# warlock-labs/sylow

Hardware: AMD Instinct MI355X
Metric: BN254 pairings/s (value) and BLS verifies/s (config.bls_verifies_per_s) at batch=2^20 per GPU (higher is better)
Workload: dtype i32/u32 limbs (9x29-bit carry-free core + 8x32-bit Montgomery, exact integer)

## Files before the change

sylow_amd/csrc/bn254_pair29.hpp:

```cpp
#pragma once
#include "bn254_f29.hpp"
#include "bn254_pair.hpp"

namespace bn254 {
namespace pl {

struct W2 { F29 c; };
BN_DEV const F29& f29_of(const W2& a) { return a.c; }
BN_DEV F29& f29_of(W2& a) { return a.c; }
struct W6 { W2 c0, c1, c2; };
struct W12 { W6 c0, c1; };

BN_DEV F29 xchg9(const F29& a) {
  F29 r;
#pragma unroll
  for (int i = 0; i < 9; ++i) r.v[i] = (i32)swap_u32((u32)a.v[i]);
  return r;
}
BN_DEV F29 sel9(bool odd, const F29& if_even, const F29& if_odd) {
  F29 r;
#pragma unroll
  for (int i = 0; i < 9; ++i) r.v[i] = odd ? if_odd.v[i] : if_even.v[i];
  return r;
}
// ... 124 lines not shown
BN_DEV W2 w2_xi_lin(const W2& x, int k, const W2& y, int m) {
  const F29 xo = xchg9(x.c);
  if (m == 0) {
    const F29* const t[2] = {&x.c, &xo};
    const i32 c[2] = {bn_keep(9 * k), bn_keep_v(lane_odd() ? k : -k)};
    return W2{f29_reduce_terms(t, c)};
  }
  const F29* const t[3] = {&x.c, &xo, &y.c};
  const i32 c[3] = {bn_keep(9 * k), bn_keep_v(lane_odd() ? k : -k), bn_keep(m)};
  return W2{f29_reduce_terms(t, c)};
}

BN_DEV W2 w2_from_s2(const S2& a) { return W2{f29_reduce(f29_from_fp(a.c))}; }
BN_DEV S2 w2_to_s2(const W2& a) { return S2{f29_to_fp(a.c)}; }
BN_DEV W2 w2_const(const uint32_t (&c)[2][8]) { return w2_from_s2(s2_const(c)); }
BN_DEV void w12_from_s12(W12& r, const S12& a) {
  r.c0.c0 = w2_from_s2(a.c0.c0); r.c0.c1 = w2_from_s2(a.c0.c1); r.c0.c2 = w2_from_s2(a.c0.c2);
  r.c1.c0 = w2_from_s2(a.c1.c0); r.c1.c1 = w2_from_s2(a.c1.c1); r.c1.c2 = w2_from_s2(a.c1.c2);
}
BN_DEV void w12_to_s12(S12& r, const W12& a) {
  r.c0.c0 = w2_to_s2(a.c0.c0); r.c0.c1 = w2_to_s2(a.c0.c1); r.c0.c2 = w2_to_s2(a.c0.c2);
  r.c1.c0 = w2_to_s2(a.c1.c0); r.c1.c1 = w2_to_s2(a.c1.c1); r.c1.c2 = w2_to_s2(a.c1.c2);
}

struct W6Raw { W2 v0, x0, y1, v2, y2; };
template <bool INL = false> BN_DEV W2 w2_mul_sel(const W2& a, const W2& b) { return INL ? w2_mul_inl(a, b) : w2_mul(a, b); }
template <bool INL = false>
BN_DEV W6Raw w6_mul_raw(const W6& a, const W6& b) {
  W2 v0, v1, v2, s0, s1, s2;
  W2_MUL2_SEL(INL, v0, v1, a.c0, b.c0, a.c1, b.c1);
  W2_MUL2_SEL(INL, v2, s0, a.c2, b.c2, w2_sub(a.c1, a.c2), w2_sub(b.c1, b.c2));
  W2_MUL2_SEL(INL, s1, s2, w2_sub(a.c0, a.c1), w2_sub(b.c0, b.c1), w2_sub(a.c0, a.c2), w2_sub(b.c0, b.c2));
  return W6Raw{v0, w2_sub(w2_add(v1, v2), s0), w2_sub(w2_add(v0, v1), s1), v2, w2_add(w2_sub(w2_add(v0, v2), s2), v1)};
}
template <bool INL = false>
BN_DEV W6 w6_mul(const W6& a, const W6& b) {
  const W6Raw m = w6_mul_raw<INL>(a, b);
  W6 r;
  r.c0 = w2_xi_lin(m.x0, 1, m.v0, 1);
  r.c1 = w2_xi_lin(m.v2, 1, m.y1, 1);
  r.c2 = w2_reduce(m.y2);
  return r;
}
BN_DEV W6 w6_add_norm(const W6& a, const W6& b) {
  return W6{w2_norm(w2_add(a.c0, b.c0)), w2_norm(w2_add(a.c1, b.c1)), w2_norm(w2_add(a.c2, b.c2))};
}
BN_DEV W6 w6_sub(const W6& a, const W6& b) { return W6{w2_sub(a.c0, b.c0), w2_sub(a.c1, b.c1), w2_sub(a.c2, b.c2)}; }

BN_DEV void w12_mul_c1(W12& r, const W6Raw& t2, const W6& t0, const W6& t1) {
  r.c1.c0 = w2_xi_lin(t2.x0, 1, w2_sub(w2_sub(t2.v0, t0.c0), t1.c0), 1);
  r.c1.c1 = w2_xi_lin(t2.v2, 1, w2_sub(w2_sub(t2.y1, t0.c1), t1.c1), 1);
  r.c1.c2 = w2_lin2(w2_sub(t2.y2, t0.c2), 1, t1.c2, -1);
}
BN_DEV W12 w12_mul(const W12& a, const W12& b) {
  const W6 t0 = w6_mul(a.c0, b.c0);
  const W6 t1 = w6_mul(a.c1, b.c1);
  const W6Raw t2 = w6_mul_raw(w6_add_norm(a.c0, a.c1), w6_add_norm(b.c0, b.c1));
  W12 r;
  w12_mul_c1(r, t2, t0, t1);
  r.c0.c0 = w2_xi_lin(t1.c2, 1, t0.c0, 1);
  r.c0.c1 = w2_norm(w2_add(t0.c1, t1.c0));
  r.c0.c2 = w2_norm(w2_add(t0.c2, t1.c1));
  return r;
}
BN_DEV W6 w6_mul_b2zero(const W6& a, const W6& b) {
  W2 v0, v1, p21, p20;
  W2_MUL2(v0, v1, a.c0, b.c0, a.c1, b.c1);
  W2_MUL2(p21, p20, a.c2, b.c1, a.c2, b.c0);
  const W2 s1 = w2_mul(w2_sub(a.c0, a.c1), w2_sub(b.c0, b.c1));
  W6 r;
  r.c0 = w2_xi_lin(p21, 1, v0, 1);
  r.c1 = w2_reduce(w2_sub(w2_add(v0, v1), s1));
  r.c2 = w2_norm(w2_add(p20, v1));
  return r;
}
BN_DEV W12 w12_mul_line_pair(const W12& a, const W12& b) {
  const W6 t0 = w6_mul(a.c0, b.c0);
  const W6 t1 = w6_mul_b2zero(a.c1, b.c1);
  const W6Raw t2 = w6_mul_raw(w6_add_norm(a.c0, a.c1), W6{w2_norm(w2_add(b.c0.c0, b.c1.c0)), w2_norm(w2_add(b.c0.c1, b.c1.c1)), b.c0.c2});
  W12 r;
  w12_mul_c1(r, t2, t0, t1);
  r.c0.c0 = w2_xi_lin(t1.c2, 1, t0.c0, 1);
  r.c0.c1 = w2_norm(w2_add(t0.c1, t1.c0));
  r.c0.c2 = w2_norm(w2_add(t0.c2, t1.c1));
  return r;
}
template <bool INL = false>
BN_DEV W12 w12_sqr(const W12& a) {
  const W6 d{w2_norm(w2_sub(a.c0.c0, a.c1.c0)), w2_norm(w2_sub(a.c0.c1, a.c1.c1)), w2_norm(w2_sub(a.c0.c2, a.c1.c2))};
  W6 e;
  e.c0 = w2_xi_lin(a.c1.c2, -1, a.c0.c0, 1);
  e.c1 = w2_norm(w2_sub(a.c0.c1, a.c1.c0));
  e.c2 = w2_norm(w2_sub(a.c0.c2, a.c1.c1));
  const W6 c2 = w6_mul<INL>(a.c0, a.c1);
  const W6Raw m = w6_mul_raw<INL>(d, e);
  W12 r;
  r.c1.c0 = w2_norm(w2_add(c2.c0, c2.c0));
  r.c1.c1 = w2_norm(w2_add(c2.c1, c2.c1));
  r.c1.c2 = w2_norm(w2_add(c2.c2, c2.c2));
  r.c0.c0 = w2_xi_lin(w2_add(m.x0, c2.c2), 1, w2_add(m.v0, c2.c0), 1);
  {
    const F29 xo = xchg9(m.v2.c);
    const W2 cc = w2_add(c2.c1, c2.c0);
    const F29* const t[4] = {&m.v2.c, &xo, &m.y1.c, &cc.c};
    const i32 c[4] = {bn_keep(9), bn_keep_v(lane_odd() ? 1 : -1), bn_keep(1), bn_keep(1)};
    r.c0.c1 = W2{f29_reduce_terms(t, c)};
  }
  r.c0.c2 = w2_lin2(m.y2, 1, w2_add(c2.c2, c2.c1), 1);
  return r;
}
BN_DEV W12 w12_conj(const W12& a) {
  W12 r;
  r.c0 = a.c0;
  r.c1.c0 = w2_norm(w2_neg(a.c1.c0)); r.c1.c1 = w2_norm(w2_neg(a.c1.c1)); r.c1.c2 = w2_norm(w2_neg(a.c1.c2));
  return r;
}
BN_DEV W2 w2_conj(const W2& a) { return W2{sel9(lane_odd(), a.c, f29_norm(f29_neg(a.c)))}; }
template <int E>
BN_DEV W6 w6_frobenius(const W6& a) {
  constexpr bool oddE = (E & 1) != 0;
  const uint32_t (&k1)[2][8] = (E == 1) ? C_FROB6_C1_1 : (E == 2) ? C_FROB6_C1_2 : C_FROB6_C1_3;
  const uint32_t (&k2)[2][8] = (E == 1) ? C_FROB6_C2_1 : (E == 2) ? C_FROB6_C2_2 : C_FROB6_C2_3;
  W6 r;
  r.c0 = oddE ? w2_conj(a.c0) : a.c0;
  W2_MUL2(r.c1, r.c2, oddE ? w2_conj(a.c1) : a.c1, w2_const(k1), oddE ? w2_conj(a.c2) : a.c2, w2_const(k2));
  return r;
}
template <int E>
BN_DEV W12 w12_frobenius(const W12& a) {
  const uint32_t (&k)[2][8] = (E == 1) ? C_FROB12_C1_1 : (E == 2) ? C_FROB12_C1_2 : C_FROB12_C1_3;
  const W2 kk = w2_const(k);
  const W6 x1 = w6_frobenius<E>(a.c1);
  W6 y;
  W2_MUL2(y.c0, y.c1, x1.c0, kk, x1.c1, kk);
  y.c2 = w2_mul(x1.c2, kk);
  return W12{w6_frobenius<E>(a.c0), y};
}
BN_DEV W12 w12_sparse_mul(const W12& f, const W2& x0, const W2& x4, const W2& x2) {
  const W2 z0 = f.c0.c0, z1 = f.c0.c1, z2 = f.c0.c2, z3 = f.c1.c0, z4 = f.c1.c1, z5 = f.c1.c2;
  W2 d0, d2, d4, p12, p54, p10, p34, p30, p52, q02, q24, q04;
  W2_MUL2(d0, d2, z0, x0, z2, x2);
  W2_MUL2(d4, p12, z4, x4, z1, x2);
  W2_MUL2(p54, p10, z5, x4, z1, x0);
  W2_MUL2(p34, p30, z3, x4, z3, x0);
  W2_MUL2(p52, q02, z5, x2, w2_sub(z0, z2), w2_sub(x0, x2));
  W2_MUL2(q24, q04, w2_sub(z2, z4), w2_sub(x2, x4), w2_sub(z0, z4), w2_sub(x0, x4));
  const W2 qs = w2_mul(w2_norm(w2_add(w2_add(z1, z3), z5)), w2_norm(w2_add(w2_add(x0, x2), x4)));
  W12 o;
  o.c0.c0 = w2_xi_lin(w2_add(p12, d4), 1, d0, 1);
  o.c0.c1 = w2_xi_lin(w2_add(p54, d2), 1, p10, 1);
  o.c0.c2 = w2_reduce(w2_add(w2_sub(w2_add(d0, d2), q02), p34));
  o.c1.c0 = w2_xi_lin(w2_sub(w2_add(d2, d4), q24), 1, p30, 1);
  o.c1.c1 = w2_xi_lin(p52, 1, w2_sub(w2_add(d0, d4), q04), 1);
  {
    const W2 sa = w2_add(w2_add(p12, p54), p10), sb = w2_add(w2_add(p34, p30), p52);
    const F29* const t[3] = {&qs.c, &sa.c, &sb.c};
    const i32 c[3] = {bn_keep(1), bn_keep(-1), bn_keep(-1)};
    o.c1.c2 = W2{f29_reduce_terms(t, c)};
  }
  return o;
}
BN_DEV W2 w2_xi_lin_v(const W2& x, const W2& y, i32 m) {
  const F29 xo = xchg9(x.c);
  const F29* const t[3] = {&x.c, &xo, &y.c};
  const i32 c[3] = {bn_keep(9), bn_keep_v(lane_odd() ? 1 : -1), bn_keep_v(m)};
  return W2{f29_reduce_terms(t, c)};
}
BN_DEV W2 w2_lin_v(const W2& x, const W2& y, i32 m) {
  const F29* const t[2] = {&x.c, &y.c};
  const i32 c[2] = {bn_keep(1), bn_keep_v(m)};
  return W2{f29_reduce_terms(t, c)};
}
BN_DEV W12 w12_sparse_mul_unit(const W12& f, i32 u, const W2& x4, const W2& x2) {
  const W2 z0 = f.c0.c0, z1 = f.c0.c1, z2 = f.c0.c2, z3 = f.c1.c0, z4 = f.c1.c1, z5 = f.c1.c2;
  W2 d2, d4, p12, p54, p34, p52, a02, a04, q24, q13;
  W2_MUL2(d2, d4, z2, x2, z4, x4);
  W2_MUL2(p12, p54, z1, x2, z5, x4);
  W2_MUL2(p34, p52, z3, x4, z5, x2);
  W2_MUL2(a02, a04, z0, x2, z0, x4);
  const W2 x24 = w2_sub(x2, x4);
  W2_MUL2(q24, q13, w2_sub(z2, z4), x24, w2_sub(z1, z3), x24);
  W12 o;
  o.c0.c0 = w2_xi_lin_v(w2_add(p12, d4), z0, u);
  o.c0.c1 = w2_xi_lin_v(w2_add(p54, d2), z1, u);
  o.c0.c2 = w2_lin_v(w2_add(a02, p34), z2, u);
  o.c1.c0 = w2_xi_lin_v(w2_sub(w2_add(d2, d4), q24), z3, u);
  {
    const F29 xo = xchg9(p52.c);
    const F29* const t[4] = {&p52.c, &xo, &a04.c, &z4.c};
    const i32 c[4] = {bn_keep(9), bn_keep_v(lane_odd() ? 1 : -1), bn_keep(1), bn_keep_v(u)};
    o.c1.c1 = W2{f29_reduce_terms(t, c)};
  }
  o.c1.c2 = w2_lin_v(w2_sub(w2_add(p12, p34), q13), z5, u);
  return o;
}
BN_DEV W2 w2_xi_norm(const W2& x, const W2& y) {
  const F29 xo = xchg9(x.c);
  const F29* const t[3] = {&x.c, &xo, &y.c};
  const i32 c[3] = {bn_keep(9), bn_keep_v(lane_odd() ? 1 : -1), bn_keep(1)};
  return W2{f29_norm_terms(t, c)};
}
BN_DEV W2 w2_xi_norm_sub(const W2& x, const W2& y) {
  const F29 xo = xchg9(x.c);
  const F29* const t[3] = {&x.c, &xo, &y.c};
  const i32 c[3] = {bn_keep(-9), bn_keep_v(lane_odd() ? -1 : 1), bn_keep(1)};
  return W2{f29_norm_terms(t, c)};
}
template <bool INL = false>
BN_DEV void w_fp4_square_fold(W2& out0, W2& m, const W2& a, const W2& b, const W2& z) {
  W2 w;
  W2_MUL2_SEL(INL, m, w, a, b, w2_sub(a, b), w2_xi_norm_sub(b, a));
  const F29 mo = xchg9(m.c);
  const F29* const t[4] = {&w.c, &m.c, &mo, &z.c};
  const i32 c[4] = {bn_keep(3), bn_keep(30), bn_keep_v(lane_odd() ? 3 : -3), bn_keep(-2)};
  out0 = W2{f29_reduce_terms(t, c)};
}
template <bool INL = false>
BN_DEV W12 w12_cyclotomic_sqr(const W12& f) {
  const W2 z0 = f.c0.c0, z4 = f.c0.c1, z3 = f.c0.c2, z2 = f.c1.c0, z1 = f.c1.c1, z5 = f.c1.c2;
  W2 m;
  W12 r;
  w_fp4_square_fold<INL>(r.c0.c0, m, z0, z1, z0);
  r.c1.c1 = w2_lin2(m, 6, z1, 2);
  w_fp4_square_fold<INL>(r.c0.c1, m, z2, z3, z4);
  r.c1.c2 = w2_lin2(m, 6, z5, 2);
  w_fp4_square_fold<INL>(r.c0.c2, m, z4, z5, z3);
  r.c1.c0 = w2_xi_lin(m, 6, z2, 2);
  return r;
}

BN_DEV F29 f29_halve(const F29& a) {
  i32 p[9]; f29_p(p);
  const i32 m = -(a.v[0] & 1);
  i32 lo[9];
  i32 c = 0;
#pragma unroll
  for (int i = 0; i < 8; ++i) {
    i32 t = a.v[i] + (p[i] & m) + c;
    lo[i] = t & BN_M29;
    c = t >> 29;
  }
  lo[8] = a.v[8] + (p[8] & m) + c;
  F29 r;
#pragma unroll
  for (int i = 0; i < 8; ++i) r.v[i] = (lo[i] >> 1) | ((lo[i + 1] & 1) << 28);
  r.v[8] = lo[8] >> 1;
  return r;
}
BN_DEV W2 w2_halve(const W2& a) { return W2{f29_halve(a.c)}; }
BN_DEV W2 w2_triple(const W2& a) { return W2{f29_add(f29_add(a.c, a.c), a.c)}; }
struct G2W { W2 x, y, z; };
BN_DEV W2 w2_twist_b() {
  const F29 k0{{0x12cb9911, 0x1fcb719e, 0x1368f727, 0x1ff96726, 0x0aadc75b, 0x179b4484, 0x06475c9b, 0x020e578d, -1520355}};
  const F29 k1{{0x0322ef99, 0x06e86c1b, 0x13f74e78, 0x0a0a4222, 0x0bcef269, 0x0af6e9ff, 0x0644c3a7, 0x0acd7c01, -535829}};
  return W2{sel9(lane_odd(), k0, k1)};
}
BN_DEV F29 f29_iso_s2() { return F29{{0x05beeef0, 0x1f76bf90, 0x1d5e46cf, 0x17f6764e, 0x1df385e5, 0x0d7a8334, 0x152215eb, 0x01b6eac1, -290196}}; }
BN_DEV F29 f29_iso_s3() { return F29{{0x1af1f8a3, 0x00cd9858, 0x1dce6a34, 0x142e620a, 0x1bc0c667, 0x0ae94d20, 0x0db9310b, 0x12572b72, 0x000405e6}}; }
BN_DEV W2 w2_mul_27m3u(const W2& a) {
  const F29 ao = xchg9(a.c);
  const F29* const t[2] = {&a.c, &ao};
  const i32 c[2] = {bn_keep(27), bn_keep_v(lane_odd() ? -3 : 3)};
  return W2{f29_reduce_terms(t, c)};
}
template <bool ISO = false>
BN_DEV void g2_doubling_step29(G2W& r, W2& l0, W2& l1, W2& l2) {
#if BN_QUAD
  W2 xy, xx, b, c, yz2, e;
  W2_MUL_SQR(xy, xx, r.x, r.y, r.x);
  const W2 a = w2_halve(xy);
  l2 = w2_norm(w2_triple(xx));
  W2_SQR2(b, c, r.y, r.z);
  if (ISO) {
    yz2 = w2_sqr(w2_norm(w2_add(r.y, r.z)));
    e = w2_mul_27m3u(c);
  } else {
    W2_SQR_MUL(yz2, e, w2_norm(w2_add(r.y, r.z)), w2_twist_b(), w2_norm(w2_triple(c)));
  }
  const W2 h = w2_norm(w2_sub(yz2, w2_add(b, c)));
  l1 = w2_neg(h);
  l0 = w2_xi_lin(w2_sub(e, b), 1, b, 0);
  const W2 f = w2_norm(w2_triple(e));
  W2_MUL2(r.z, r.x, b, h, a, w2_sub(b, f));
  const W2 g = w2_halve(w2_norm(w2_add(b, f)));
  W2 gg, ee;
  W2_SQR2(gg, ee, g, e);
  r.y = w2_lin2(gg, 1, ee, -3);
#else
  const W2 a = w2_halve(w2_mul(r.x, r.y));
  l2 = w2_norm(w2_triple(w2_sqr(r.x)));
  const W2 b = w2_sqr(r.y);
  const W2 c = w2_sqr(r.z);
  const W2 h = w2_norm(w2_sub(w2_sqr(w2_norm(w2_add(r.y, r.z))), w2_add(b, c)));
  const W2 e = ISO ? w2_mul_27m3u(c) : w2_mul(w2_twist_b(), w2_norm(w2_triple(c)));
  l1 = w2_neg(h);
  r.z = w2_mul(b, h);
  l0 = w2_xi_lin(w2_sub(e, b), 1, b, 0);
  const W2 f = w2_norm(w2_triple(e));
  r.x = w2_mul(a, w2_sub(b, f));
  const W2 g = w2_halve(w2_norm(w2_add(b, f)));
  r.y = w2_lin2(w2_sqr(g), 1, w2_sqr(e), -3);
#endif
}
BN_DEV void g2_addition_step29(G2W& r, const W2& bx, const W2& by, W2& l0, W2& l1, W2& l2) {
#if BN_QUAD
  W2 zbx, zby, ebx, dby;
  W2_MUL2(zbx, zby, r.z, bx, r.z, by);
  const W2 d = w2_sub(r.x, zbx);
  const W2 e = w2_sub(r.y, zby);
  W2_MUL2(ebx, dby, e, bx, d, by);
  l0 = w2_xi_lin(w2_sub(ebx, dby), 1, bx, 0);
  l1 = d;
  l2 = w2_neg(e);
  const W2 dn = w2_norm(d), en = w2_norm(e);
  W2 f, ee, h, i, zee, zh, dj, hy;
  W2_SQR2(f, ee, dn, en);
  W2_MUL2(h, i, dn, f, r.x, f);
  W2_MUL2(zee, zh, r.z, ee, r.z, h);
  const W2 j = w2_norm(w2_sub(w2_add(zee, h), w2_add(i, i)));
  W2_MUL2(dj, hy, dn, j, h, r.y);
  r.z = zh;
  r.x = dj;
  r.y = w2_norm(w2_sub(w2_mul(en, w2_sub(i, j)), hy));
#else
  const W2 d = w2_sub(r.x, w2_mul(r.z, bx));
  const W2 e = w2_sub(r.y, w2_mul(r.z, by));
  l0 = w2_xi_lin(w2_sub(w2_mul(e, bx), w2_mul(d, by)), 1, bx, 0);
  l1 = d;
  l2 = w2_neg(e);
  const W2 dn = w2_norm(d), en = w2_norm(e);
  const W2 f = w2_sqr(dn);
  const W2 h = w2_mul(dn, f);
  const W2 i = w2_mul(r.x, f);
  const W2 j = w2_norm(w2_sub(w2_add(w2_mul(r.z, w2_sqr(en)), h), w2_add(i, i)));
  r.z = w2_mul(r.z, h);
  r.x = w2_mul(dn, j);
  r.y = w2_norm(w2_sub(w2_mul(en, w2_sub(i, j)), w2_mul(h, r.y)));
#endif
}
BN_DEV W12 w12_line_product(const W2& a0, const W2& a4, const W2& a2, const W2& b0, const W2& b4, const W2& b2) {
  W2 d0, d2, d4, k02, k24, k04;
  W2_MUL2(d0, d2, a0, b0, a2, b2);
  W2_MUL2(d4, k02, a4, b4, w2_sub(a0, a2), w2_sub(b0, b2));
  W2_MUL2(k24, k04, w2_sub(a2, a4), w2_sub(b2, b4), w2_sub(a0, a4), w2_sub(b0, b4));
  W12 r;
  r.c0.c0 = w2_xi_lin(d4, 1, d0, 1);
  r.c0.c1 = w2_xi_lin(d2, 1, d2, 0);
  r.c0.c2 = w2_reduce(w2_sub(w2_add(d0, d2), k02));
  r.c1.c0 = w2_xi_lin(w2_sub(w2_add(d2, d4), k24), 1, d2, 0);
  r.c1.c1 = w2_reduce(w2_sub(w2_add(d0, d4), k04));
  r.c1.c2 = W2{F29{{0, 0, 0, 0, 0, 0, 0, 0, 0}}};
  return r;
}
constexpr int MILLER_LDS_WORDS = 36, MILLER_LDS_WORDS_PARK = 63;
BN_DEV void lds_put9(i32 (*lds)[256], int slot, const F29& a) {
#pragma unroll
  for (int i = 0; i < 9; ++i) lds[9 * slot + i][threadIdx.x] = a.v[i];
}
BN_DEV F29 lds_get9(i32 (*lds)[256], int slot) {
  F29 r;
#pragma unroll
  for (int i = 0; i < 9; ++i) r.v[i] = lds[9 * slot + i][threadIdx.x];
  return r;
}
#ifndef BN_MILLER_SQR_INL
#define BN_MILLER_SQR_INL false
#endif
template <bool PARK, bool ISO = false>
BN_NOINLINE void miller_loop29g(S12& fout, const Fp& pxs, const Fp& pys, const S2& qxs_in, const S2& qys_in) {
  __shared__ i32 lds[PARK ? MILLER_LDS_WORDS_PARK : MILLER_LDS_WORDS][256];
  S2 qxs = qxs_in, qys = qys_in;
  {
    const F29 px = f29_reduce(f29_from_fp(pxs)), py = f29_reduce(f29_from_fp(pys));
    lds_put9(lds, 0, ISO ? f29_mul(px, f29_iso_s2()) : px);
    lds_put9(lds, 1, ISO ? f29_mul(py, f29_iso_s3()) : py);
  }
  {
    W2 qx = w2_from_s2(qxs), qy = w2_from_s2(qys);
    if (ISO) {
      W2_SCALE2(qx, qy, qx, f29_iso_s2(), qy, f29_iso_s3());
      qxs = w2_to_s2(qx); qys = w2_to_s2(qy);
    }
    lds_put9(lds, 2, qx.c);
    lds_put9(lds, 3, qy.c);
  }
  auto PX = [&]() { return lds_get9(lds, 0); };
  auto PY = [&]() { return lds_get9(lds, 1); };
  auto QX = [&]() { return W2{lds_get9(lds, 2)}; };
  auto QY = [&](bool neg) { const W2 y{lds_get9(lds, 3)}; return neg ? w2_neg(y) : y; };
  auto park = [&](const G2W& r) { if (PARK) { lds_put9(lds, 4, r.x.c); lds_put9(lds, 5, r.y.c); lds_put9(lds, 6, r.z.c); } };
  auto unpark = [&](const G2W& r) { return PARK ? G2W{W2{lds_get9(lds, 4)}, W2{lds_get9(lds, 5)}, W2{lds_get9(lds, 6)}} : r; };
  W12 f;
  G2W r{QX(), QY(false), w2_from_s2(s2_one())};
  W2 l0, l1, l2;
  auto line_mul = [&](const W12& x) {
    W2 s1, s2;
    W2_SCALE2(s1, s2, l1, PY(), l2, PX());
    return w12_sparse_mul(x, l0, s1, s2);
  };
  const u64 nz = BN_ATE_NAF_NZ, ng = BN_ATE_NAF_NEG;
  static_assert((BN_ATE_NAF_NZ >> 63) & 1, "the first digit of 6x+2 after the leading one is non-zero");
  {
    g2_doubling_step29<ISO>(r, l0, l1, l2);
    const W2 d0 = l0;
    W2 d4, d2, e4, e2;
    W2_SCALE2(d4, d2, l1, PY(), l2, PX());
    g2_addition_step29(r, QX(), QY((ng >> 63) & 1), l0, l1, l2);
    park(r);
    W2_SCALE2(e4, e2, l1, PY(), l2, PX());
    f = w12_line_product(d0, d4, d2, l0, e4, e2);
  }
#pragma unroll 1
  for (int i = 1; i < 64; ++i) {
    r = unpark(r);
    g2_doubling_step29<ISO>(r, l0, l1, l2);
    park(r);
    f = w12_sqr<BN_MILLER_SQR_INL>(f);
    f = line_mul(f);
    if ((nz >> (63 - i)) & 1) {
      r = unpark(r);
      g2_addition_step29(r, QX(), QY((ng >> (63 - i)) & 1), l0, l1, l2);
      park(r);
      f = line_mul(f);
    }
  }
  r = unpark(r);
  S2 q1x, q1y, q2x, q2y;
  g2_psi_affine(q1x, q1y, qxs, qys);
  g2_psi_affine(q2x, q2y, q1x, q1y);
  q2y = s2_neg(q2y);
  g2_addition_step29(r, w2_from_s2(q1x), w2_from_s2(q1y), l0, l1, l2);
  f = line_mul(f);
  g2_addition_step29(r, w2_from_s2(q2x), w2_from_s2(q2y), l0, l1, l2);
  f = line_mul(f);
  w12_to_s12(fout, f);
}


BN_DEV void w12_pin(W12& x) {
  W2* const c[6] = {&x.c0.c0, &x.c0.c1, &x.c0.c2, &x.c1.c0, &x.c1.c1, &x.c1.c2};
#pragma unroll
  for (int j = 0; j < 6; ++j)
#pragma unroll
    for (int i = 0; i < 9; ++i) BN_CHAIN_NV(c[j]->c.v[i]);
}
BN_NOINLINE void w12_mul_nl(W12& r, const W12& a, const W12& b) {
  W12 x = a, y = b;
  w12_pin(x); w12_pin(y);
  r = w12_mul(x, y);
}
BN_NOINLINE void w12_cyclotomic_sqr_nl(W12& r, const W12& a) {
  W12 x = a;
  w12_pin(x);
  r = w12_cyclotomic_sqr(x);
}
template <int E> BN_NOINLINE void w12_frobenius_nl(W12& r, const W12& a) {
  W12 x = a;
  w12_pin(x);
  r = w12_frobenius<E>(x);
}
#ifndef BN_EXP_INL
#define BN_EXP_INL true
#endif
#define BN_X_C_NZ 0x0008144402208421ull
#define BN_X_C_NEG 0x0008004400000020ull
#define BN_X_C_17 0x0000100000008021ull
BN_NOINLINE void exp_by_neg_z29(W12& r, const W12& f) {
  W12 tab[2];
  {
    W12 t, u;
    w12_cyclotomic_sqr_nl(t, f);
    w12_cyclotomic_sqr_nl(u, t);
    w12_cyclotomic_sqr_nl(t, u);
    w12_cyclotomic_sqr_nl(u, t);
    w12_mul_nl(tab[0], u, f);
    w12_cyclotomic_sqr_nl(t, tab[0]);
    w12_mul_nl(tab[1], t, f);
  }
  W12 res = tab[1];
  const u64 nz = BN_X_C_NZ, ng = BN_X_C_NEG, i17 = BN_X_C_17;
#pragma unroll 1
  for (int i = 56; i >= 0; --i) {
    res = w12_cyclotomic_sqr<BN_EXP_INL>(res);
    if ((nz >> i) & 1) {
      W12 m = tab[((i17 >> i) & 1) ? 0 : 1];
      if ((ng >> i) & 1) m = w12_conj(m);
      res = w12_mul(res, m);
    }
  }
  r = w12_conj(res);
}
BN_DEV W2 w2_inv(const W2& a) {
  const F29 t = f29_mul_leaf(W_ARGS(a.c), W_ARGS(a.c));
  const F29 n = f29_norm(f29_add(t, xchg9(t)));
  const F29 i = f29_reduce(f29_from_fp(fp_inv(f29_to_fp(n))));
  const F29 r = f29_mul_leaf(W_ARGS(a.c), W_ARGS(i));
  return W2{sel9(lane_odd(), r, f29_norm(f29_neg(r)))};
}
BN_DEV W2 w2_mul_xi(const W2& a) { return w2_xi_lin(a, 1, a, 0); }
BN_DEV W6 w6_inv(const W6& a) {
  W2 s0, m12, s2, m01, s1, m02, u1, u2, o0, o1;
  W2_SQR_MUL(s0, m12, a.c0, a.c1, w2_mul_xi(a.c2));
  W2_SQR_MUL(s2, m01, a.c2, a.c0, a.c1);
  W2_SQR_MUL(s1, m02, a.c1, a.c0, a.c2);
  const W2 t0 = w2_sub(s0, m12);
  const W2 t1 = w2_sub(w2_mul_xi(s2), m01);
  const W2 t2 = w2_sub(s1, m02);
  W2_MUL2(u1, u2, a.c2, t1, a.c1, t2);
  const W2 d = w2_xi_lin(w2_add(u1, u2), 1, w2_mul(a.c0, t0), 1);
  const W2 di = w2_inv(d);
  W2_MUL2(o0, o1, di, t0, di, t1);
  return W6{o0, o1, w2_mul(di, t2)};
}
BN_NOINLINE void w12_inv_nl(W12& r, const W12& ain) {
  W12 a = ain;
  w12_pin(a);
  const W6 s0 = w6_mul(a.c0, a.c0), s1 = w6_mul(a.c1, a.c1);
  const W6 d{w2_norm(w2_sub(s0.c0, w2_mul_xi(s1.c2))), w2_norm(w2_sub(s0.c1, s1.c0)), w2_norm(w2_sub(s0.c2, s1.c1))};
  const W6 t = w6_inv(d);
  r.c0 = w6_mul(a.c0, t);
  const W6 m = w6_mul(a.c1, t);
  r.c1 = W6{w2_norm(w2_neg(m.c0)), w2_norm(w2_neg(m.c1)), w2_norm(w2_neg(m.c2))};
}
BN_NOINLINE void final_exponentiation29(S12& out, const S12& fin) {
  W12 in, t, a, b, d, e, g;
  {
    w12_from_s12(t, fin);
    w12_inv_nl(b, t);
    a = w12_conj(t);
    w12_mul_nl(d, a, b);
    w12_frobenius_nl<2>(a, d);
    w12_mul_nl(in, a, d);
  }
  exp_by_neg_z29(a, in);
  w12_cyclotomic_sqr_nl(b, a);
  w12_cyclotomic_sqr_nl(t, b);
  w12_mul_nl(d, t, b);
  exp_by_neg_z29(e, d);
  w12_cyclotomic_sqr_nl(t, e);
  exp_by_neg_z29(g, t);
  d = w12_conj(d);
  g = w12_conj(g);
  w12_mul_nl(t, g, e);
  w12_mul_nl(a, t, d);
  w12_mul_nl(d, a, b);
  w12_mul_nl(t, a, e);
  w12_mul_nl(e, in, t);
  w12_frobenius_nl<1>(t, d);
  w12_mul_nl(b, t, e);
  w12_frobenius_nl<2>(t, a);
  w12_mul_nl(e, t, b);
  t = w12_conj(in);
  w12_mul_nl(a, t, d);
  w12_frobenius_nl<3>(t, a);
  w12_mul_nl(g, t, e);
  w12_to_s12(out, g);
}


#ifdef BN_WIDE_LEAF_CALL
BN_DEV W2 w2_mul_w(const W2& a, const W2& b) { return w2_mul(a, b); }
#else
BN_DEV W2 w2_mul_w(const W2& a, const W2& b) { return w2_mul_inl(a, b); }
#endif
struct alignas(16) WideLds { i32 v[63][2][12]; };
typedef __attribute__((address_space(3))) WideLds* WideLdsPtr;
template <int EPW> BN_DEV int wide_j(int lane) { return (int)pair_index((u32)lane) & (32 / EPW - 1); }
typedef i32 __attribute__((ext_vector_type(4))) WideVec4;
typedef __attribute__((address_space(3))) WideVec4* WideVec4Ptr;
BN_DEV void wide_put(WideLdsPtr x, int slot, int odd, const W2& a) {
  const WideVec4Ptr p = (WideVec4Ptr)&x->v[slot][odd][0];
  p[0] = WideVec4{a.c.v[0], a.c.v[1], a.c.v[2], a.c.v[3]};
  p[1] = WideVec4{a.c.v[4], a.c.v[5], a.c.v[6], a.c.v[7]};
  x->v[slot][odd][8] = a.c.v[8];
}
BN_DEV W2 wide_get(WideLdsPtr x, int slot, int odd) {
  const WideVec4Ptr p = (WideVec4Ptr)&x->v[slot][odd][0];
  const WideVec4 lo = p[0], hi = p[1];
  W2 r;
  r.c.v[0] = lo.x; r.c.v[1] = lo.y; r.c.v[2] = lo.z; r.c.v[3] = lo.w;
  r.c.v[4] = hi.x; r.c.v[5] = hi.y; r.c.v[6] = hi.z; r.c.v[7] = hi.w;
  r.c.v[8] = x->v[slot][odd][8];
  return r;
}
BN_DEV W2 w2_pick(const W2& a, const W2& b, bool c) { return W2{sel9(c, a.c, b.c)}; }
BN_DEV W2 w2_real(const F29& k) { return W2{sel9(lane_odd(), k, F29{{0, 0, 0, 0, 0, 0, 0, 0, 0}})}; }
BN_DEV W2 w2_sel3(int k, const W2& a, const W2& b, const W2& c) { return w2_pick(w2_pick(a, b, k == 1), c, k == 2); }
template <int EPW = 1>
BN_DEV W12 w12_cyclotomic_sqr_wide(const W12& f, WideLdsPtr x) {
  const int lane = (int)(threadIdx.x & 63u), odd = pair_role((u32)lane), j = wide_j<EPW>(lane);
  const int p = j < 6 ? j : 0, k = p >> 1;
  const bool s = (p & 1) != 0;
  const W2 z0 = f.c0.c0, z4 = f.c0.c1, z3 = f.c0.c2, z2 = f.c1.c0, z1 = f.c1.c1, z5 = f.c1.c2;
  const W2 a = w2_sel3(k, z0, z2, z4), b = w2_sel3(k, z1, z3, z5);
  {
    const W2 xs = w2_pick(a, w2_norm(w2_add(a, b)), s), ys = w2_pick(b, w2_xi_norm(b, a), s);
    const W2 pr = w2_mul_w(xs, ys);
    if (j < 6) wide_put(x, p, odd, pr);
  }
  __syncthreads();
  {
    const int ko = p < 2 ? 0 : p < 4 ? 2 : 1;
    const bool ta = p == 0 || p == 3 || p == 4, tc = p == 2;
    const W2 m = wide_get(x, 2 * ko, odd), w = wide_get(x, 2 * ko + 1, odd);
    const W2 z = w2_pick(a, b, s);
    const F29 mo = xchg9(m.c);
    const bool lo = lane_odd();
    const F29* const t[4] = {&w.c, &m.c, &mo, &z.c};
    const i32 c[4] = {bn_keep_v(ta ? 3 : 0), bn_keep_v(ta ? -30 : tc ? 54 : 6), bn_keep_v(ta ? (lo ? -3 : 3) : tc ? (lo ? 6 : -6) : 0), bn_keep_v(ta ? -2 : 2)};
    const W2 r{f29_reduce_terms(t, c)};
    if (j < 6) wide_put(x, 6 + (p < 2 ? p : p < 4 ? p + 2 : p - 2), odd, r);
  }
  __syncthreads();
  W12 r;
  r.c0.c0 = wide_get(x, 6, odd); r.c1.c1 = wide_get(x, 7, odd); r.c0.c1 = wide_get(x, 8, odd);
  r.c1.c2 = wide_get(x, 9, odd); r.c1.c0 = wide_get(x, 10, odd); r.c0.c2 = wide_get(x, 11, odd);
  return r;
}
constexpr int WL_IA = 12, WL_IB = 18, WL_SA = 24, WL_SB = 27, WL_P = 30, WL_T = 48, WL_OUT = 57;
constexpr int WK_DENSE = 0, WK_LINE = 1, WK_SQUARE = 2;
#ifndef BN_WIDE_MILLER_INL
#define BN_WIDE_MILLER_INL 2
#endif
#ifndef BN_WIDE_KINDS
#define BN_WIDE_KINDS 1
#endif
BN_DEV W2 w12_coef(const W12& a, int c) {
  const W2 lo = w2_sel3(c % 3, a.c0.c0, a.c0.c1, a.c0.c2), hi = w2_sel3(c % 3, a.c1.c0, a.c1.c1, a.c1.c2);
  return w2_pick(lo, hi, c >= 3);
}
template <int EPW = 1, int KIND = WK_DENSE>
BN_DEV void w12_mul_wide_stage0(const W12& a, const W12& b, WideLdsPtr x) {
  const int lane = (int)(threadIdx.x & 63u), odd = pair_role((u32)lane), j = wide_j<EPW>(lane);
  {
    const int c = j < 6 ? j : 0;
    const int i = c % 3;
    const W2 a0i = w2_sel3(i, a.c0.c0, a.c0.c1, a.c0.c2), a1i = w2_sel3(i, a.c1.c0, a.c1.c1, a.c1.c2);
    const W2 sa = w2_norm(w2_add(a0i, a1i));
    if (KIND == WK_SQUARE) {
      const W2 sb0 = w2_xi_lin(a.c1.c2, 1, a.c0.c0, 1);
      const W2 sb12 = w2_norm(w2_add(a0i, w2_pick(a.c1.c0, a.c1.c1, i == 2)));
      if (j < 3) { wide_put(x, WL_IA + i, odd, a0i); wide_put(x, WL_IB + i, odd, a1i); wide_put(x, WL_SA + i, odd, sa); }
      if (j >= 3 && j < 6) wide_put(x, WL_SB + i, odd, w2_pick(sb12, sb0, i == 0));
    } else {
      const W2 ac = w2_pick(a0i, a1i, c >= 3), bc = w12_coef(b, c);
      const W2 sb = w2_norm(w2_add(w2_sel3(i, b.c0.c0, b.c0.c1, b.c0.c2), w2_sel3(i, b.c1.c0, b.c1.c1, b.c1.c2)));
      if (j < 6) { wide_put(x, WL_IA + c, odd, ac); wide_put(x, WL_IB + c, odd, bc); }
      if (j < 3) wide_put(x, WL_SA + i, odd, sa);
      if (j >= 3 && j < 6) wide_put(x, WL_SB + i, odd, sb);
    }
  }
}
template <int EPW = 1, int KIND = WK_DENSE, bool STAGE3 = true>
BN_DEV void w12_mul_wide_core(WideLdsPtr x) {
  const int lane = (int)(threadIdx.x & 63u), odd = pair_role((u32)lane), j = wide_j<EPW>(lane);
  const W2 zero{F29{{0, 0, 0, 0, 0, 0, 0, 0, 0}}};
  __syncthreads();
#pragma unroll
  for (int pass = 0; pass < (KIND == WK_DENSE ? EPW : 1); ++pass) {
    int w;
    bool live;
    if (KIND == WK_DENSE) {
      const int jw = j + 16 * pass;
      live = jw < 18;
      w = live ? jw : 0;
    } else if (KIND == WK_LINE) {
      live = j < 14;
      w = live ? j + (j >= 1) + (j >= 5) + (j >= 6) + (j >= 8) : 0;
    } else {
      live = j < 12;
      w = j < 6 ? j : live ? j + 6 : 0;
    }
    const int g = w / 6, h = w % 6;
    const int i0 = h < 3 ? h : h == 3 ? 1 : 0, i1 = h < 3 ? h : h == 4 ? 1 : 2;
    const int ba = g == 0 ? WL_IA : g == 1 ? WL_IA + 3 : WL_SA, bb = g == 0 ? WL_IB : g == 1 ? WL_IB + 3 : WL_SB;
    const W2 xa = wide_get(x, ba + i0, odd), xb = wide_get(x, ba + i1, odd);
    const W2 ya = wide_get(x, bb + i0, odd), yb = wide_get(x, bb + i1, odd);
    const W2 xs = w2_pick(xa, w2_norm(w2_add(xa, xb)), h >= 3), ys = w2_pick(ya, w2_norm(w2_add(ya, yb)), h >= 3);
    const W2 pr = w2_mul_w(xs, ys);
    if (live) wide_put(x, WL_P + w, odd, pr);
    if (KIND == WK_LINE && j < 4) wide_put(x, WL_P + (int)((0x0B080601u >> (8 * j)) & 255u), odd, zero);
  }
  __syncthreads();
  {
    const int nu = KIND == WK_SQUARE ? 6 : 9;
    const int u = j >= nu ? 0 : (KIND == WK_SQUARE && j >= 3) ? j + 3 : j, g = u / 3, c = u % 3, base = WL_P + 6 * g;
    const W2 v0 = wide_get(x, base, odd), v1 = wide_get(x, base + 1, odd), v2 = wide_get(x, base + 2, odd), q = wide_get(x, base + 3 + c, odd);
    const W2 xv = w2_pick(v2, w2_sub(w2_sub(q, v1), v2), c == 0);
    const F29 xo = xchg9(xv.c);
    const bool lo = lane_odd();
    const F29* const t[6] = {&xv.c, &xo, &q.c, &v0.c, &v1.c, &v2.c};
    const i32 kx = c == 2 ? 0 : 1;
    const i32 k[6] = {bn_keep_v(9 * kx), bn_keep_v(lo ? kx : -kx), bn_keep_v(c == 0 ? 0 : 1), bn_keep_v(c == 0 ? 1 : -1),
                      bn_keep_v(c == 0 ? 0 : c == 1 ? -1 : 1), bn_keep_v(c == 2 ? -1 : 0)};
    if (j < nu) wide_put(x, WL_T + u, odd, W2{f29_reduce_terms(t, k)});
  }
  __syncthreads();
  if (!STAGE3) return;
  if (KIND == WK_SQUARE) {
    const int o = j < 6 ? j : 0, i = o % 3;
    const W2 ti = wide_get(x, WL_T + i, odd), tp = wide_get(x, WL_T + (i + 2) % 3, odd), mi = wide_get(x, WL_T + 6 + i, odd);
    const F29 tpo = xchg9(tp.c);
    const bool lo = lane_odd(), hi = o >= 3, o0 = o == 0;
    const F29* const t[4] = {&ti.c, &tp.c, &tpo, &mi.c};
    const i32 k[4] = {bn_keep_v(hi ? 2 : -1), bn_keep_v(hi ? 0 : o0 ? -9 : -1), bn_keep_v(o0 ? (lo ? -1 : 1) : 0), bn_keep_v(hi ? 0 : 1)};
    if (j < 6) wide_put(x, WL_OUT + o, odd, W2{f29_reduce_terms(t, k)});
  } else {
    const int o = j < 6 ? j : 0, i = o % 3;
    const int pa = o >= 3 ? i : o, pb = o >= 3 ? 3 + i : o == 0 ? 5 : o == 1 ? 3 : 4, pc = o >= 3 ? 6 + i : 0;
    const W2 ta = wide_get(x, WL_T + pa, odd), tb = wide_get(x, WL_T + pb, odd), tc = wide_get(x, WL_T + pc, odd);
    const F29 tbo = xchg9(tb.c);
    const bool lo = lane_odd(), hi = o >= 3, o0 = o == 0;
    const F29* const t[4] = {&ta.c, &tb.c, &tbo, &tc.c};
    const i32 k[4] = {bn_keep_v(hi ? -1 : 1), bn_keep_v(hi ? -1 : o0 ? 9 : 1), bn_keep_v(o0 ? (lo ? 1 : -1) : 0), bn_keep_v(hi ? 1 : 0)};
    if (j < 6) wide_put(x, WL_OUT + o, odd, W2{f29_reduce_terms(t, k)});
  }
  __syncthreads();
}
BN_DEV W12 w12_wide_result(WideLdsPtr x) {
  const int odd = pair_role((u32)(threadIdx.x & 63u));
  W12 r;
  r.c0.c0 = wide_get(x, WL_OUT, odd); r.c0.c1 = wide_get(x, WL_OUT + 1, odd); r.c0.c2 = wide_get(x, WL_OUT + 2, odd);
  r.c1.c0 = wide_get(x, WL_OUT + 3, odd); r.c1.c1 = wide_get(x, WL_OUT + 4, odd); r.c1.c2 = wide_get(x, WL_OUT + 5, odd);
  return r;
}
template <int EPW = 1, int KIND = WK_DENSE>
BN_DEV W12 w12_mul_wide(const W12& a, const W12& b, WideLdsPtr x) {
  w12_mul_wide_stage0<EPW, KIND>(a, b, x);
  w12_mul_wide_core<EPW, KIND>(x);
  return w12_wide_result(x);
}
template <int EPW = 1, int KIND = WK_DENSE>
BN_NOINLINE void w12_mul_wide_core_nl(WideLds* xg) { w12_mul_wide_core<EPW, KIND>((WideLdsPtr)xg); }
template <int EPW = 1, int KIND = WK_DENSE>
BN_DEV void w12_mul_wide_nl(W12& r, const W12& a, const W12& b, WideLds* xg) {
  w12_mul_wide_stage0<EPW, KIND>(a, b, (WideLdsPtr)xg);
  w12_mul_wide_core_nl<EPW, KIND>(xg);
  r = w12_wide_result((WideLdsPtr)xg);
}
template <int EPW = 1>
BN_NOINLINE void exp_by_neg_z29_wide(W12& r, const W12& f, WideLds* xg) {
  const WideLdsPtr x = (WideLdsPtr)xg;
  W12 tab[2];
  {
    W12 t = f;
#pragma unroll 1
    for (int k = 0; k < 5; ++k) {
      t = w12_cyclotomic_sqr_wide<EPW>(t, x);
      if (k == 3) {
        w12_mul_wide_nl<EPW>(tab[0], t, f, xg);
        t = tab[0];
      }
    }
    w12_mul_wide_nl<EPW>(tab[1], t, f, xg);
  }
  W12 res = tab[1];
  const u64 nz = BN_X_C_NZ, ng = BN_X_C_NEG, i17 = BN_X_C_17;
#pragma unroll 1
  for (int i = 56; i >= 0; --i) {
    res = w12_cyclotomic_sqr_wide<EPW>(res, x);
    if ((nz >> i) & 1) {
      W12 m = tab[((i17 >> i) & 1) ? 0 : 1];
      if ((ng >> i) & 1) m = w12_conj(m);
      res = w12_mul_wide<EPW>(res, m, x);
    }
  }
  r = w12_conj(res);
}
template <int E, int EPW = 1>
BN_DEV W12 w12_frobenius_wide(const W12& a, WideLdsPtr x) {
  constexpr bool oddE = (E & 1) != 0;
  const int lane = (int)(threadIdx.x & 63u), odd = pair_role((u32)lane), j = wide_j<EPW>(lane);
  const W2 k1 = w2_const((E == 1) ? C_FROB6_C1_1 : (E == 2) ? C_FROB6_C1_2 : C_FROB6_C1_3);
  const W2 k2 = w2_const((E == 1) ? C_FROB6_C2_1 : (E == 2) ? C_FROB6_C2_2 : C_FROB6_C2_3);
  const W2 kk = w2_const((E == 1) ? C_FROB12_C1_1 : (E == 2) ? C_FROB12_C1_2 : C_FROB12_C1_3);
  {
    const int p = j < 5 ? j : 0;
    const W2 c = w2_pick(w2_pick(w2_pick(w2_pick(a.c0.c1, a.c0.c2, p == 1), a.c1.c0, p == 2), a.c1.c1, p == 3), a.c1.c2, p == 4);
    const W2 u = oddE ? w2_conj(c) : c;
    const W2 v = w2_pick(w2_pick(k1, k2, p == 1 || p == 4), kk, p == 2);
    const W2 pr = w2_mul_w(u, v);
    if (j < 5) wide_put(x, WL_P + p, odd, pr);
  }
  __syncthreads();
  {
    const W2 u = wide_get(x, WL_P + 3 + (j == 1 ? 1 : 0), odd);
    const W2 pr = w2_mul_w(u, kk);
    if (j < 2) wide_put(x, WL_T + j, odd, pr);
  }
  __syncthreads();
  W12 r;
  r.c0.c0 = oddE ? w2_conj(a.c0.c0) : a.c0.c0;
  r.c0.c1 = wide_get(x, WL_P, odd); r.c0.c2 = wide_get(x, WL_P + 1, odd);
  r.c1.c0 = wide_get(x, WL_P + 2, odd); r.c1.c1 = wide_get(x, WL_T, odd); r.c1.c2 = wide_get(x, WL_T + 1, odd);
  return r;
}
template <int EPW>
BN_DEV void w6_mul2_wide(const W6& a, const W6& b, const W6& c, const W6& d, WideLdsPtr x) {
  const int lane = (int)(threadIdx.x & 63u), odd = pair_role((u32)lane), j = wide_j<EPW>(lane);
  const int i = (j < 6 ? j : 0) % 3;
  const bool hi = j >= 3;
  const W2 u = w2_sel3(i, w2_pick(a.c0, c.c0, hi), w2_pick(a.c1, c.c1, hi), w2_pick(a.c2, c.c2, hi));
  const W2 v = w2_sel3(i, w2_pick(b.c0, d.c0, hi), w2_pick(b.c1, d.c1, hi), w2_pick(b.c2, d.c2, hi));
  if (j < 3) { wide_put(x, WL_IA + i, odd, u); wide_put(x, WL_IB + i, odd, v); }
  if (j >= 3 && j < 6) { wide_put(x, WL_SA + i, odd, u); wide_put(x, WL_SB + i, odd, v); }
  w12_mul_wide_core<EPW, WK_SQUARE, false>(x);
}
BN_DEV W6 w6_wide_t(WideLdsPtr x, int base) {
  const int odd = pair_role((u32)(threadIdx.x & 63u));
  return W6{wide_get(x, WL_T + base, odd), wide_get(x, WL_T + base + 1, odd), wide_get(x, WL_T + base + 2, odd)};
}
template <int EPW = 1>
BN_DEV W12 w12_inv_wide(const W12& a, WideLdsPtr x) {
  const int lane = (int)(threadIdx.x & 63u), odd = pair_role((u32)lane), j = wide_j<EPW>(lane);
  w6_mul2_wide<EPW>(a.c0, a.c0, a.c1, a.c1, x);
  const W6 s0 = w6_wide_t(x, 0), s1 = w6_wide_t(x, 6);
  const W2 d0 = w2_norm(w2_sub(s0.c0, w2_mul_xi(s1.c2))), d1 = w2_norm(w2_sub(s0.c1, s1.c0)), d2 = w2_norm(w2_sub(s0.c2, s1.c1));
  {
    const int p = j < 6 ? j : 0;
    const W2 xd2 = w2_mul_xi(d2);
    const W2 u = w2_pick(w2_pick(d0, d1, p == 1 || p == 4), d2, p == 2);
    const W2 v = w2_pick(w2_pick(w2_pick(w2_pick(d0, xd2, p == 1), d2, p == 2 || p == 5), d1, p == 3 || p == 4), d0, p == 0);
    const W2 pr = w2_mul_w(u, v);
    if (j < 6) wide_put(x, WL_P + p, odd, pr);
  }
  __syncthreads();
  const W2 t0 = w2_sub(wide_get(x, WL_P, odd), wide_get(x, WL_P + 1, odd));
  const W2 t1 = w2_sub(w2_mul_xi(wide_get(x, WL_P + 2, odd)), wide_get(x, WL_P + 3, odd));
  const W2 t2 = w2_sub(wide_get(x, WL_P + 4, odd), wide_get(x, WL_P + 5, odd));
  {
    const int p = j < 3 ? j : 0;
    const W2 pr = w2_mul_w(w2_sel3(p, d2, d1, d0), w2_sel3(p, t1, t2, t0));
    if (j < 3) wide_put(x, WL_P + 6 + p, odd, pr);
  }
  __syncthreads();
  const W2 dd = w2_xi_lin(w2_add(wide_get(x, WL_P + 6, odd), wide_get(x, WL_P + 7, odd)), 1, wide_get(x, WL_P + 8, odd), 1);
  const W2 di = w2_inv(dd);
  {
    const int p = j < 3 ? j : 0;
    const W2 pr = w2_mul_w(di, w2_sel3(p, t0, t1, t2));
    if (j < 3) wide_put(x, WL_P + 9 + p, odd, pr);
  }
  __syncthreads();
  const W6 t{wide_get(x, WL_P + 9, odd), wide_get(x, WL_P + 10, odd), wide_get(x, WL_P + 11, odd)};
  w6_mul2_wide<EPW>(a.c0, t, a.c1, t, x);
  const W6 m = w6_wide_t(x, 6);
  W12 r;
  r.c0 = w6_wide_t(x, 0);
  r.c1 = W6{w2_norm(w2_neg(m.c0)), w2_norm(w2_neg(m.c1)), w2_norm(w2_neg(m.c2))};
  return r;
}
template <int EPW = 1>
BN_NOINLINE void final_exponentiation29_wide(S12& out, const S12& fin, WideLds* x) {
  W12 in, t, a, b, d, e, g;
  {
    w12_from_s12(t, fin);
    b = w12_inv_wide<EPW>(t, (WideLdsPtr)x);
    a = w12_conj(t);
    w12_mul_wide_nl<EPW>(d, a, b, x);
    a = w12_frobenius_wide<2, EPW>(d, (WideLdsPtr)x);
// ... 156 lines not shown
```

sylow_amd/csrc/plk_verify_body.hpp:

```cpp
#pragma once
#include "plk_common.hpp"

namespace plk {
BN_DEV void stage_table(i32* lds, const i32* src) {
  for (int k = threadIdx.x; k < LINE_TABLE_WORDS; k += blockDim.x) lds[k] = src[k];
}
BN_DEV W2 table_w2(const i32* tab, int at, int c, int odd) {
  const i32* t = tab + ((at * 2 + c) * 2 + odd) * 9;
  return W2{F29{{t[0], t[1], t[2], t[3], t[4], t[5], t[6], t[7], t[8]}}};
}
BN_DEV i32 table_unit(const i32* tab, int at) { return tab[LINE_TABLE_LINES * 36 + at]; }

template <bool PK_TABLE>
BN_DEV void bls_verify_fused_body(const u64* pkxy, const uint8_t* pkinf, const i32* pk_table,
                                  const u64* hneg, const uint8_t* hneg_inf,
                                  const u64* sigxy, const uint8_t* siginf, const i32* gen_table, uint8_t* okout, size_t n, size_t m, const Stagger& st) {
  __shared__ i32 tabA[LINE_TABLE_WORDS];
  __shared__ i32 tabB[PK_TABLE ? LINE_TABLE_WORDS : 1];
  unsigned chunk;
  int role = stagger_role(st, chunk);
  const size_t t = (size_t)chunk * blockDim.x + threadIdx.x, i = elem_index(t);
  const int odd = pair_role(t);
  const size_t np = (size_t)st.count * ELEMS_PER_BLOCK, ip = (size_t)(chunk - st.first) * ELEMS_PER_BLOCK + (i & (ELEMS_PER_BLOCK - 1));
  if (role == 2 && !stagger_wait(st, chunk)) role = 0;
  if (role == 2) {
    S12 fs, g;
    load_s12(fs, st.park, np, ip, odd);
    final_exponentiation29(g, fs);
    const bool one = s12_is_one(g);
    if (!odd && elem_writer(t)) okout[i] = one ? 1 : 0;
    return;
  }
  stage_table(tabA, gen_table);
  if (PK_TABLE) stage_table(tabB, pk_table);
  __syncthreads();
  const bool active = i < m;
  const size_t ii = active ? i : 0;
  const Fp hxs = load_fp(hneg, n, ii, 0), hys = load_fp(hneg, n, ii, 4);
  const bool hinf = hneg_inf[ii] != 0;
  __shared__ i32 lds[PK_TABLE ? 36 : 54][256];
  const bool liveA = !(siginf && siginf[ii]);
  const bool liveB = !(hinf || (pkinf && pkinf[PK_TABLE ? 0 : ii]));
  const F29 f29_zero{{0, 0, 0, 0, 0, 0, 0, 0, 0}};
  lds_put9(lds, 0, liveA ? f29_reduce(f29_from_fp(load_fp(sigxy, n, ii, 0))) : f29_zero);
  lds_put9(lds, 1, liveA ? f29_reduce(f29_from_fp(load_fp(sigxy, n, ii, 4))) : f29_zero);
  constexpr bool ISO = !PK_TABLE;
  lds_put9(lds, 2, liveB ? (ISO ? f29_mul(f29_reduce(f29_from_fp(hxs)), f29_iso_s2()) : f29_reduce(f29_from_fp(hxs))) : f29_zero);
  lds_put9(lds, 3, liveB ? (ISO ? f29_mul(f29_reduce(f29_from_fp(hys)), f29_iso_s3()) : f29_reduce(f29_from_fp(hys))) : f29_zero);
  auto SX = [&]() { return lds_get9(lds, 0); };
  auto SY = [&]() { return lds_get9(lds, 1); };
  auto HX = [&]() { return lds_get9(lds, 2); };
  auto HY = [&]() { return lds_get9(lds, 3); };
  auto key_x = [&]() { return (PK_TABLE || !liveB) ? s2_g2gen_x() : load_s2(pkxy, n, ii, 0, odd); };
  auto key_y = [&]() { return (PK_TABLE || !liveB) ? s2_g2gen_y() : load_s2(pkxy, n, ii, 8, odd); };
  G2W r;
  {
    W2 qx = w2_from_s2(key_x()), qy = w2_from_s2(key_y());
    if (ISO) W2_SCALE2(qx, qy, qx, f29_iso_s2(), qy, f29_iso_s3());
    if (!PK_TABLE) { lds_put9(lds, 4, qx.c); lds_put9(lds, 5, qy.c); }
    r = G2W{qx, qy, w2_from_s2(s2_one())};
  }
  auto QX = [&]() { return W2{lds_get9(lds, PK_TABLE ? 0 : 4)}; };
  auto QY = [&](bool neg) {
    const W2 y{lds_get9(lds, PK_TABLE ? 0 : 5)};
    return neg ? w2_neg(y) : y;
  };
  W12 f;
  {
    S12 one = s12_one();
    w12_from_s12(f, one);
  }
  W2 l0, l1, l2;
  int idx = 0;
  auto lineA = [&]() {
    W2 a1, a2;
    W2_SCALE2(a1, a2, table_w2(tabA, idx, 0, odd), SY(), table_w2(tabA, idx, 1, odd), SX());
    f = w12_sparse_mul_unit(f, liveA ? table_unit(tabA, idx) : 1, a1, a2);
  };
  auto lineB = [&]() {
    if (PK_TABLE) {
      W2 b1, b2;
      W2_SCALE2(b1, b2, table_w2(tabB, idx, 0, odd), HY(), table_w2(tabB, idx, 1, odd), HX());
      f = w12_sparse_mul_unit(f, liveB ? table_unit(tabB, idx) : 1, b1, b2);
    } else {
      W2 s1, s2;
      W2_SCALE2(s1, s2, l1, HY(), l2, HX());
      f = w12_sparse_mul(f, l0, s1, s2);
    }
  };
  const u64 nz = BN_ATE_NAF_NZ, ng = BN_ATE_NAF_NEG;
#pragma unroll 1
  for (int it = 0; it < 64; ++it) {
    f = w12_sqr(f);
    lineA();
    if (!PK_TABLE) g2_doubling_step29<ISO>(r, l0, l1, l2);
    lineB();
    ++idx;
    if ((nz >> (63 - it)) & 1) {
      lineA();
      if (!PK_TABLE) g2_addition_step29(r, QX(), QY(((ng >> (63 - it)) & 1) != 0), l0, l1, l2);
      lineB();
      ++idx;
    }
  }
  S2 q1x, q1y, q2x, q2y;
  if (!PK_TABLE) { g2_psi_affine(q1x, q1y, w2_to_s2(QX()), w2_to_s2(QY(false))); g2_psi_affine(q2x, q2y, q1x, q1y); }
  lineA();
  if (!PK_TABLE) g2_addition_step29(r, w2_from_s2(q1x), w2_from_s2(q1y), l0, l1, l2);
  lineB();
  ++idx;
  lineA();
  if (!PK_TABLE) g2_addition_step29(r, w2_from_s2(q2x), w2_from_s2(s2_neg(q2y)), l0, l1, l2);
  lineB();
  S12 fs, g;
  w12_to_s12(fs, f);
  if (role == 1) {
    store_s12(st.park, np, ip, odd, fs);
    stagger_publish(st, chunk);
    return;
  }
  final_exponentiation29(g, fs);
  const bool one = s12_is_one(g);
  if (active && !odd && elem_writer(t)) okout[i] = one ? 1 : 0;
}
}
```

Baseline: 9.621 million.

## Peel first Miller iteration, skip final point update and last FE multiply

```diff
diff --git a/sylow_amd/csrc/bn254_pair29.hpp b/sylow_amd/csrc/bn254_pair29.hpp
--- a/sylow_amd/csrc/bn254_pair29.hpp
+++ b/sylow_amd/csrc/bn254_pair29.hpp
@@ -450,6 +450,7 @@
   r.y = w2_lin2(w2_sqr(g), 1, w2_sqr(e), -3);
 #endif
 }
+template <bool LINE_ONLY = false>
 BN_DEV void g2_addition_step29(G2W& r, const W2& bx, const W2& by, W2& l0, W2& l1, W2& l2) {
 #if BN_QUAD
   W2 zbx, zby, ebx, dby;
@@ -460,6 +461,7 @@
   l0 = w2_xi_lin(w2_sub(ebx, dby), 1, bx, 0);
   l1 = d;
   l2 = w2_neg(e);
+  if (LINE_ONLY) return;
   const W2 dn = w2_norm(d), en = w2_norm(e);
   W2 f, ee, h, i, zee, zh, dj, hy;
   W2_SQR2(f, ee, dn, en);
@@ -476,6 +478,7 @@
   l0 = w2_xi_lin(w2_sub(w2_mul(e, bx), w2_mul(d, by)), 1, bx, 0);
   l1 = d;
   l2 = w2_neg(e);
+  if (LINE_ONLY) return;
   const W2 dn = w2_norm(d), en = w2_norm(e);
   const W2 f = w2_sqr(dn);
   const W2 h = w2_mul(dn, f);
@@ -670,7 +673,8 @@
   const W6 m = w6_mul(a.c1, t);
   r.c1 = W6{w2_norm(w2_neg(m.c0)), w2_norm(w2_neg(m.c1)), w2_norm(w2_neg(m.c2))};
 }
-BN_NOINLINE void final_exponentiation29(S12& out, const S12& fin) {
+template <bool IS_ONE>
+BN_DEV bool final_exponentiation29_impl(S12* out, const S12& fin) {
   W12 in, t, a, b, d, e, g;
   {
     w12_from_s12(t, fin);
@@ -701,9 +705,26 @@
   t = w12_conj(in);
   w12_mul_nl(a, t, d);
   w12_frobenius_nl<3>(t, a);
+  if (IS_ONE) {
+    S12 x, y;
+    w12_to_s12(x, t);
+    w12_to_s12(y, w12_conj(e));
+    const S2* const xc[6] = {&x.c0.c0, &x.c0.c1, &x.c0.c2, &x.c1.c0, &x.c1.c1, &x.c1.c2};
+    const S2* const yc[6] = {&y.c0.c0, &y.c0.c1, &y.c0.c2, &y.c1.c0, &y.c1.c1, &y.c1.c2};
+    bool eq = true, zero = true;
+#pragma unroll
+    for (int j = 0; j < 6; ++j) {
+      eq = eq & s2_eq(*xc[j], *yc[j]);
+      zero = zero & s2_is_zero(*xc[j]);
+    }
+    return eq && !zero;
+  }
   w12_mul_nl(g, t, e);
-  w12_to_s12(out, g);
-}
+  w12_to_s12(*out, g);
+  return false;
+}
+BN_NOINLINE void final_exponentiation29(S12& out, const S12& fin) { final_exponentiation29_impl<false>(&out, fin); }
+BN_NOINLINE bool final_exponentiation29_is_one(const S12& fin) { return final_exponentiation29_impl<true>(nullptr, fin); }
 
 
 #ifdef BN_WIDE_LEAF_CALL
diff --git a/sylow_amd/csrc/plk_verify_body.hpp b/sylow_amd/csrc/plk_verify_body.hpp
--- a/sylow_amd/csrc/plk_verify_body.hpp
+++ b/sylow_amd/csrc/plk_verify_body.hpp
@@ -24,10 +24,9 @@
   const size_t np = (size_t)st.count * ELEMS_PER_BLOCK, ip = (size_t)(chunk - st.first) * ELEMS_PER_BLOCK + (i & (ELEMS_PER_BLOCK - 1));
   if (role == 2 && !stagger_wait(st, chunk)) role = 0;
   if (role == 2) {
-    S12 fs, g;
+    S12 fs;
     load_s12(fs, st.park, np, ip, odd);
-    final_exponentiation29(g, fs);
-    const bool one = s12_is_one(g);
+    const bool one = final_exponentiation29_is_one(fs);
     if (!odd && elem_writer(t)) okout[i] = one ? 1 : 0;
     return;
   }
@@ -66,12 +65,15 @@
     return neg ? w2_neg(y) : y;
   };
   W12 f;
-  {
-    S12 one = s12_one();
-    w12_from_s12(f, one);
-  }
   W2 l0, l1, l2;
   int idx = 0;
+  auto unit_w2 = [&](i32 u) {
+    const W2 one = w2_from_s2(s2_one());
+    W2 w;
+#pragma unroll
+    for (int k = 0; k < 9; ++k) w.c.v[k] = u ? one.c.v[k] : 0;
+    return w;
+  };
   auto lineA = [&]() {
     W2 a1, a2;
     W2_SCALE2(a1, a2, table_w2(tabA, idx, 0, odd), SY(), table_w2(tabA, idx, 1, odd), SX());
@@ -89,8 +91,27 @@
     }
   };
   const u64 nz = BN_ATE_NAF_NZ, ng = BN_ATE_NAF_NEG;
+  static_assert((BN_ATE_NAF_NZ >> 63) & 1, "the first digit of 6x+2 after the leading one is non-zero");
+  {
+    W2 a1, a2, b0, b1, b2;
+    W2_SCALE2(a1, a2, table_w2(tabA, idx, 0, odd), SY(), table_w2(tabA, idx, 1, odd), SX());
+    if (PK_TABLE) {
+      W2_SCALE2(b1, b2, table_w2(tabB, idx, 0, odd), HY(), table_w2(tabB, idx, 1, odd), HX());
+      b0 = unit_w2(liveB ? table_unit(tabB, idx) : 1);
+    } else {
+      g2_doubling_step29<ISO>(r, l0, l1, l2);
+      W2_SCALE2(b1, b2, l1, HY(), l2, HX());
+      b0 = l0;
+    }
+    f = w12_line_product(unit_w2(liveA ? table_unit(tabA, idx) : 1), a1, a2, b0, b1, b2);
+    ++idx;
+    lineA();
+    if (!PK_TABLE) g2_addition_step29(r, QX(), QY(((ng >> 63) & 1) != 0), l0, l1, l2);
+    lineB();
+    ++idx;
+  }
 #pragma unroll 1
-  for (int it = 0; it < 64; ++it) {
+  for (int it = 1; it < 64; ++it) {
     f = w12_sqr(f);
     lineA();
     if (!PK_TABLE) g2_doubling_step29<ISO>(r, l0, l1, l2);
@@ -110,17 +131,16 @@
   lineB();
   ++idx;
   lineA();
-  if (!PK_TABLE) g2_addition_step29(r, w2_from_s2(q2x), w2_from_s2(s2_neg(q2y)), l0, l1, l2);
+  if (!PK_TABLE) g2_addition_step29<true>(r, w2_from_s2(q2x), w2_from_s2(s2_neg(q2y)), l0, l1, l2);
   lineB();
-  S12 fs, g;
+  S12 fs;
   w12_to_s12(fs, f);
   if (role == 1) {
     store_s12(st.park, np, ip, odd, fs);
     stagger_publish(st, chunk);
     return;
   }
-  final_exponentiation29(g, fs);
-  const bool one = s12_is_one(g);
+  const bool one = final_exponentiation29_is_one(fs);
   if (active && !odd && elem_writer(t)) okout[i] = one ? 1 : 0;
 }
 }
```

After: 9.629 million, median of 4. About the same (+0.1%).
